# eBay/Sequence-Semantic-Embedding

Measured on AMD Instinct MI355X. Metric: encoded seqs/sec (+ query x target cosine-scores/sec, top-1 vs ref), higher is better.
Workload: dtype f32; 1 GPU; configs[1]: classification stand-in, dual-encoder LSTM H=S=256 E=50 T=32 V=32000; encode 16384 source seqs/GPU/step + cosine top-10 vs 571-target index; batch_per_gpu=16384, seq_len=32, targets=571, parallelism=dp1, weights=random-init (reference initialisers, seed 0)

## Files before the change

### sequence-semantic-embedding_amd/csrc/score_topk.hip

```cpp
#include <cstdlib>

#include "sse_kernels.h"
#include "score_exact.h"

#define SC_THREADS 512
#define SC_KC 16
#ifndef SC_PRIO_K
#define SC_PRIO_K 1
#define SC_PRIO_E 0
#endif

#ifdef SSE_SCORE_CLOCK
#include <cstdio>
__device__ long long g_score_clk[8 * 8];
#define SC_CLK_DECL long long ck_[8] = {0, 0, 0, 0, 0, 0, 0, 0}, ck_t = clock64();
#define SC_CLK(i)                   \
  {                                 \
    const long long n_ = clock64(); \
    ck_[i] += n_ - ck_t;            \
    ck_t = n_;                      \
  }
#else
#define SC_CLK_DECL
#define SC_CLK(i)
// ... 834 lines not shown
__device__ __forceinline__ float wave_max_f(float x) {
  x = fmaxf(x, dpp_f<0x128, 0xF>(x));
  x = fmaxf(x, dpp_f<0x124, 0xF>(x));
  x = fmaxf(x, dpp_f<0x122, 0xF>(x));
  x = fmaxf(x, dpp_f<0x121, 0xF>(x));
  x = fmaxf(x, dpp_f<0x142, 0xA>(x));
  x = fmaxf(x, dpp_f<0x143, 0xC>(x));
  return __int_as_float(__builtin_amdgcn_readlane(__float_as_int(x), 63));
}
template <int JMAX>
#ifdef SSE_SCORE_CLOCK
#define SI_CLK_PARAMS , long long (&ck_)[8], long long &ck_t
#define SI_CLK_ARGS , ck_, ck_t
#else
#define SI_CLK_PARAMS
#define SI_CLK_ARGS
#endif
__device__ __forceinline__ void si_select4(const SmallIndexArgs &a, const float *sc, int NP, int NT, int qt, int q0, int lane SI_CLK_PARAMS) {
  constexpr int QW = 4;
  const int J = (NT * 32 + 63) / 64;
  float v[QW][JMAX];
#pragma unroll
  for (int j = 0; j < JMAX; ++j) {
    const int row = lane + 64 * j;
#pragma unroll
    for (int c = 0; c < QW; ++c) v[c][j] = (j < J && row < NT * 32) ? sc[(q0 + c) * NP + row] : NEG_INF;
  }
  int lok[QW], hik[QW];
  float lm[QW];
  bool done[QW];
#pragma unroll
  for (int c = 0; c < QW; ++c) {
    float m = NEG_INF;
#pragma unroll
    for (int j = 0; j < JMAX; ++j) m = fmaxf(m, v[c][j]);
    lm[c] = m;
    lok[c] = si_key(-wave_max_f(-m));
    hik[c] = si_key(wave_max_f(m)) + 1;
    done[c] = false;
  }
  SC_CLK(5)
  for (;;) {
    bool all_done = true;
#pragma unroll
    for (int c = 0; c < QW; ++c) {
      const unsigned width = (unsigned)hik[c] - (unsigned)lok[c];
      const int mid = lok[c] + (int)(width >> 1);
      const int cnt = __popcll(__ballot(lm[c] >= si_val(mid)));
      const bool open = !done[c] && width > 1u;
      const bool ge = cnt >= SC_KC;
      lok[c] = (open && ge) ? mid : lok[c];
      hik[c] = (open && !ge) ? mid : hik[c];
      done[c] = !open || (ge && cnt <= 24);
      all_done = all_done && done[c];
    }
    if (all_done) break;
  }
  SC_CLK(6)
#pragma unroll
  for (int c = 0; c < QW; ++c) {
    const int query = qt * 32 + q0 + c;
    if (query < a.Q) {
      const float T = si_val(lok[c]);
      float cs = NEG_INF;
      int cr = -1, base = 0;
#pragma unroll
      for (int j = 0; j < JMAX; ++j) {
        const bool take = (j < J) & (v[c][j] >= T) & (v[c][j] > NEG_INF);
        const unsigned long long mask = __ballot(take);
        const int n = __popcll(mask);
        const int slot = base + (int)__builtin_amdgcn_mbcnt_hi((unsigned)(mask >> 32), __builtin_amdgcn_mbcnt_lo((unsigned)mask, 0u));
        const int dst = (take && slot < 63) ? slot : 63;
        const int gs = __builtin_amdgcn_ds_permute(dst * 4, __float_as_int(v[c][j]));
        const int gr = __builtin_amdgcn_ds_permute(dst * 4, lane + 64 * j);
        const bool recv = (lane >= base) & (lane < base + n) & (lane < 63);
        cs = recv ? __int_as_float(gs) : cs;
        cr = recv ? gr : cr;
        base += n;
      }
      const int nw = base < 63 ? base : 63;
      int rank = 0;
      for (int l = 0; l < nw; ++l) {
        const float os = __int_as_float(__builtin_amdgcn_readlane(__float_as_int(cs), l));
        const int orow = __builtin_amdgcn_readlane(cr, l);
        rank += ((os > cs) | ((os == cs) & (orow < cr))) ? 1 : 0;
      }
      const bool mine = lane < nw;
      if (mine && rank < SC_KC) {
        a.part_scores[(size_t)query * SC_KC + rank] = cs;
        a.part_ids[(size_t)query * SC_KC + rank] = cr;
      }
      if (lane >= nw && lane < SC_KC) {
        a.part_scores[(size_t)query * SC_KC + lane] = NEG_INF;
        a.part_ids[(size_t)query * SC_KC + lane] = -1;
      }
      const unsigned long long m16 = __ballot(mine && rank == SC_KC - 1);
      const float last = m16 ? __int_as_float(__builtin_amdgcn_readlane(__float_as_int(cs), __ffsll((long long)m16) - 1)) : NEG_INF;
      if (lane == 0) a.part_bnd[query] = (base > 63) ? __builtin_inff() : last;
    }
  }
}

template <int KGC>
__global__ __launch_bounds__(256) void score_small_index_kernel(SmallIndexArgs a) {
  extern __shared__ __attribute__((aligned(16))) float si_sc[];
  const int tid = threadIdx.x, lane = tid & 63, w = __builtin_amdgcn_readfirstlane(tid >> 6);
  const int NT = a.NT, NP = NT * 32 + 1;
  const int qt = blockIdx.x;
  float *sc = si_sc;
  SC_CLK_DECL
  f32x4 b[KGC];
  {
    const int row = qt * 32 + (lane & 31), kb = (lane >> 5) * 4;
    const float *src = a.q_rows + (size_t)(row < a.Q ? row : 0) * a.S + kb;
    const bool vec = (a.S & 3) == 0 && (reinterpret_cast<uintptr_t>(a.q_rows) & 15) == 0 && KGC * 8 <= a.S;
#pragma unroll
    for (int kg = 0; kg < KGC; ++kg) {
      f32x4 v = {0, 0, 0, 0};
      if (vec) {
        v = *reinterpret_cast<const f32x4 *>(src + kg * 8);
      } else {
#pragma unroll
        for (int e = 0; e < 4; ++e)
          if (kg * 8 + kb + e < a.S) v[e] = src[kg * 8 + e];
      }
      if (row >= a.Q) v = f32x4{0, 0, 0, 0};
      b[kg] = v;
    }
  }
  SC_CLK(0)
  for (int t = w; t < NT; t += 4) {
    const f32x4 *ap = reinterpret_cast<const f32x4 *>(a.idxp) + (size_t)t * KGC * 64 + lane;
    f32x16 acc = {0, 0, 0, 0, 0, 0, 0, 0, 0, 0, 0, 0, 0, 0, 0, 0};
    f32x4 ar[4];
#pragma unroll
    for (int d = 0; d < 4; ++d) ar[d] = ap[(d < KGC ? d : 0) * 64];
#pragma unroll
    for (int kg = 0; kg < KGC; ++kg) {
      __builtin_amdgcn_sched_barrier(0);
#pragma unroll
      for (int e = 0; e < 4; ++e) acc = __builtin_amdgcn_mfma_f32_32x32x2f32(ar[kg & 3][e], b[kg][e], acc, 0, 0, 0);
      __builtin_amdgcn_sched_barrier(0);
      ar[kg & 3] = ap[(kg + 4 < KGC ? kg + 4 : kg) * 64];
    }
    const int rb = t * 32 + 4 * (lane >> 5);
    float *col = sc + (lane & 31) * NP;
#pragma unroll
    for (int r = 0; r < 16; ++r) {
      const int row = rb + (r & 3) + 8 * (r >> 2);
      col[row] = (row < a.N) ? acc[r] : NEG_INF;
    }
  }
  SC_CLK(1)
  __syncthreads();
  SC_CLK(2)
  if (NT * 32 <= 640) {
    si_select4<10>(a, sc, NP, NT, qt, w * 8, lane SI_CLK_ARGS);
    SC_CLK(3)
    si_select4<10>(a, sc, NP, NT, qt, w * 8 + 4, lane SI_CLK_ARGS);
    SC_CLK(4)
#ifdef SSE_SCORE_CLOCK
    if (blockIdx.x == gridDim.x / 2 && lane == 0)
      for (int i = 0; i < 8; ++i) g_score_clk[w * 8 + i] = ck_[i];
#endif
  } else {
    si_select4<16>(a, sc, NP, NT, qt, w * 8, lane SI_CLK_ARGS);
    si_select4<16>(a, sc, NP, NT, qt, w * 8 + 4, lane SI_CLK_ARGS);
  }
// ... 91 lines not shown
bool score_small_index_applies(int Q, int KG, int64_t NT) {
  return Q >= 1024 && (KG == 32 || KG == 8 || KG == 7) && NT * 32 <= 1024 && (size_t)32 * (NT * 32 + 1) * sizeof(float) <= (size_t)144 * 1024;
}
hipError_t launch_score_small_index(const SmallIndexArgs &a, hipStream_t stream) {
  if (!score_small_index_applies(a.Q, a.KG, a.NT)) return hipErrorInvalidValue;
  const size_t lds = (size_t)32 * (a.NT * 32 + 1) * sizeof(float);
  const dim3 grid((a.Q + 31) / 32), block(256);
  auto go = [&](auto kernel) -> hipError_t {
    hipError_t e = hipFuncSetAttribute(reinterpret_cast<const void *>(kernel), hipFuncAttributeMaxDynamicSharedMemorySize, (int)lds);
    if (e != hipSuccess) return e;
    hipLaunchKernelGGL(kernel, grid, block, lds, stream, a);
    return hipGetLastError();
  };
  if (a.idx_x3 && a.KG != 32) return go(score_small_index_x3_kernel<4>);
  if (a.KG == 8) return go(score_small_index_kernel<8>);
  if (a.KG == 7) return go(score_small_index_kernel<7>);
  const hipError_t e32 = a.idx_x3 ? go(score_small_index_x3_kernel<16>) : go(score_small_index_kernel<32>);
  if (e32 != hipSuccess) return e32;
#ifdef SSE_SCORE_CLOCK
  if (a.Q >= 8192) {
    static int n = 0;
    if (n++ % 8 == 3) {
      long long v[64];
      (void)hipStreamSynchronize(stream);
      (void)hipMemcpyFromSymbol(v, HIP_SYMBOL(g_score_clk), sizeof v);
      for (int w = 0; w < 4; w += 3)
        fprintf(stderr, "[small index clock Q=%d NT=%d] wave %d cycles: query fragments %lld | scores (MFMA + LDS stores) %lld | barrier %lld | selection: loads + bounds %lld | bisection %lld | winners + rank + stores %lld (both batches)\n",
                a.Q, a.NT, w, v[w * 8 + 0], v[w * 8 + 1], v[w * 8 + 2], v[w * 8 + 5], v[w * 8 + 6], v[w * 8 + 3] + v[w * 8 + 4]);
    }
  }
#endif
  return hipGetLastError();
}

hipError_t launch_score_topk(const ScoreArgs &a_in, hipStream_t stream) {
  ScoreArgs a = a_in;
#ifdef SSE_SCORE_MEASURE
  {
    static const int dbg = getenv("SSE_SCORE_DBG") ? atoi(getenv("SSE_SCORE_DBG")) : 0;
    a.dbg = dbg;
  }
#endif
  if (a.KC != SC_KC) return hipErrorInvalidValue;
  if (a.q_rows && ((a.NQ != 1 && !a.COLLECT) || a.S < 1)) return hipErrorInvalidValue;
  if (a.NSPLIT > 8 && (a.NSPLIT & 7)) return hipErrorInvalidValue;
  if (a.NSPLIT < 8 && (8 % a.NSPLIT)) return hipErrorInvalidValue;
  if (a.COLLECT) {
    if (!a.lane_max && (!a.col_thr || !a.col_slot || !a.col_cnt || !a.col_buf)) return hipErrorInvalidValue;
    if (a.BF) return a.NQ == 4 ? launch_score_variant<4, true, true>(a, stream) : hipErrorInvalidValue;
    if (a.NQ == 1) return launch_score_variant<1, false, true>(a, stream);
    if (a.NQ == 2) return launch_score_variant<2, false, true>(a, stream);
    if (a.NQ == 4) return launch_score_variant<4, false, true>(a, stream);
    return hipErrorInvalidValue;
  }
  if (!a.part_bnd) return hipErrorInvalidValue;
  if (a.BF) {
    if (a.NQ == 1) return launch_score_variant<1, true, false>(a, stream);
    if (a.NQ == 2) return launch_score_variant<2, true, false>(a, stream);
    if (a.NQ == 4) return launch_score_variant<4, true, false>(a, stream);
    return hipErrorInvalidValue;
  }
  if (a.NQ == 1) return launch_score_variant<1, false, false>(a, stream);
  if (a.NQ == 2) return launch_score_variant<2, false, false>(a, stream);
  if (a.NQ == 4) return launch_score_variant<4, false, false>(a, stream);
  return hipErrorInvalidValue;
}


template <int NB>
__device__ __forceinline__ int packed_value_of_lane(int lane) {
  int v = 0;
#pragma unroll
  for (int cnt = NB, bit = 5; cnt > 1; cnt >>= 1, --bit) v = v * 2 + ((lane >> bit) & 1);
  return v;
}
template <int NB>
__device__ __forceinline__ int packed_lane_of_value(int v) {
  int lane = 0;
#pragma unroll
  for (int cnt = NB, bit = 5; cnt > 1; cnt >>= 1, --bit) lane |= ((v / (cnt / 2)) & 1) << bit;
  return lane;
}
template <int NB>
__device__ __forceinline__ double wave_exact_dot_packed(const float *qrow, const float *idxp, const double *idx64, const int64_t (&n)[NB],
                                                        int S, int KG, int lane, const float *idx_rm = nullptr) {
  static_assert(NB == 2 || NB == 4 || NB == 8, "power of two");
  double acc[NB];
#pragma unroll
  for (int b = 0; b < NB; ++b) acc[b] = 0.0;
  if (idx64) {
    for (int d = lane; d < S; d += 64) {
      double rv[NB];
#pragma unroll
      for (int b = 0; b < NB; ++b) rv[b] = idx64[(size_t)n[b] * S + d];
#pragma unroll
      for (int b = 0; b < NB; ++b) acc[b] += (double)qrow[d] * rv[b];
    }
  } else {
    for (int j = lane; j < KG * 2; j += 64) {
      const int kg = j >> 1, half = j & 1;
      f32x4 v[NB];
#pragma unroll
      for (int b = 0; b < NB; ++b)
        v[b] = idx_rm ? *reinterpret_cast<const f32x4 *>(idx_rm + (size_t)n[b] * S + j * 4)
                      : *reinterpret_cast<const f32x4 *>(idxp + (size_t)(n[b] >> 5) * KG * 256 + kg * 256 + (half * 32 + (int)(n[b] & 31)) * 4);
      const int d0 = kg * 8 + half * 4;
#pragma unroll
      for (int e = 0; e < 4; ++e)
        if (d0 + e < S) {
#pragma unroll
          for (int b = 0; b < NB; ++b) acc[b] += (double)qrow[d0 + e] * (double)v[b][e];
        }
    }
  }
  int m = 32;
#pragma unroll
  for (int cnt = NB; cnt > 1; cnt >>= 1, m >>= 1) {
    const bool up = (lane & m) != 0;
#pragma unroll
    for (int i = 0; i < cnt / 2; ++i) {
      const double send = up ? acc[i] : acc[i + cnt / 2];
      const double keep = up ? acc[i + cnt / 2] : acc[i];
      acc[i] = keep + __shfl_xor(send, m);
    }
  }
#pragma unroll
  for (; m > 0; m >>= 1) acc[0] += __shfl_xor(acc[0], m);
  return acc[0];
}

#define RS_THREADS 256
#define RS_MAXWIN 256
#define RS_MAXNC 4096
__global__ __launch_bounds__(RS_THREADS) void rescore_kernel(RescoreArgs a) {
  __shared__ int s_cnt;
  __shared__ int s_wid[RS_MAXWIN];
  __shared__ double s_ex[RS_MAXWIN];
  __shared__ float s_m[RS_THREADS / 64];
  __shared__ double s_qn[RS_THREADS / 64];
  extern __shared__ __attribute__((aligned(16))) unsigned long long s_key[];
  const int q = blockIdx.x, tid = threadIdx.x, lane = tid & 63, w = tid >> 6;
  if (a.uncert_clear && q == 0 && tid == 0) *a.uncert_clear = 0;
  if (a.q_count && q >= *a.q_count) return;
  const int qo = a.qmap ? a.qmap[q] : q;
  const float *ps = a.part_scores + (size_t)q * a.NC;
  const int32_t *pi = a.part_ids + (size_t)q * a.NC;
  const float *qrow = a.q + (size_t)q * a.S;
  const int KG = (a.S + 7) / 8;

  constexpr int PER = RS_MAXNC / RS_THREADS;
  float rs[PER];
  int ri[PER];
#pragma unroll
  for (int j = 0; j < PER; ++j) {
    const int c = tid + j * RS_THREADS;
    ri[j] = (c < a.NC) ? pi[c] : -1;
    rs[j] = (c < a.NC) ? ps[c] : NEG_INF;
  }
  float mmax = NEG_INF;
  for (int c = tid; c < a.NC / SC_KC; c += RS_THREADS) mmax = fmaxf(mmax, a.part_bnd[(size_t)q * (a.NC / SC_KC) + c]);

  {
    double v = 0.0;
    for (int d = tid; d < a.S; d += RS_THREADS) v += (double)qrow[d] * qrow[d];
#pragma unroll
    for (int o = 32; o > 0; o >>= 1) v += __shfl_xor(v, o);
    if (lane == 0) s_qn[w] = v;
  }
#pragma unroll
  for (int o = 32; o > 0; o >>= 1) mmax = fmaxf(mmax, __shfl_xor(mmax, o));
  if (lane == 0) s_m[w] = mmax;
  if (tid == 0) s_cnt = 0;

#pragma unroll
  for (int j = 0; j < PER; ++j) {
    const int c = tid + j * RS_THREADS;
    if (c < a.NC) {
      unsigned u = __float_as_uint(rs[j]);
      u = (u & 0x80000000u) ? ~u : (u | 0x80000000u);
      s_key[c] = (ri[j] < 0) ? 0ull : (((unsigned long long)u << 32) | (unsigned long long)(0xFFFFFFFFu - (unsigned)ri[j]));
    }
  }
  __syncthreads();
  const float qnorm = (float)sqrt(s_qn[0] + s_qn[1] + s_qn[2] + s_qn[3]);
  const float eps_q = a.eps * qnorm;
  mmax = fmaxf(fmaxf(s_m[0], s_m[1]), fmaxf(s_m[2], s_m[3]));
  float kth = NEG_INF;
  if (a.NC <= 256) {
    const unsigned long long key = (tid < a.NC) ? s_key[tid] : 0ull;
    int rank = 0;
    for (int j = 0; j < a.NC; ++j) rank += (s_key[j] > key) ? 1 : 0;
    float mine = (key != 0ull && rank == a.k - 1) ? rs[0] : NEG_INF;
#pragma unroll
    for (int o = 32; o > 0; o >>= 1) mine = fmaxf(mine, __shfl_xor(mine, o));
    __shared__ float s_thr[RS_THREADS / 64];
    if (lane == 0) s_thr[w] = mine;
    __syncthreads();
    kth = fmaxf(fmaxf(s_thr[0], s_thr[1]), fmaxf(s_thr[2], s_thr[3]));
  } else {
    __shared__ unsigned long long s_best[(RS_THREADS / 64) * SC_KC];
    const int nslots = a.NC / SC_KC;
    int head[RS_MAXNC / SC_KC / RS_THREADS];
#pragma unroll
    for (int j = 0; j < RS_MAXNC / SC_KC / RS_THREADS; ++j) head[j] = 0;
    for (int it = 0; it < a.k; ++it) {
      unsigned long long best = 0ull;
#pragma unroll
      for (int j = 0; j < RS_MAXNC / SC_KC / RS_THREADS; ++j) {
        const int slot = tid + j * RS_THREADS;
        if (slot < nslots && head[j] < SC_KC) {
          const unsigned long long key = s_key[slot * SC_KC + head[j]];
// ... 28 lines not shown
    for (int o = 32; o > 0; o >>= 1) {
      const unsigned long long other = __shfl_xor(kkey, o);
      kkey = other > kkey ? other : kkey;
    }
    if (kkey != 0ull) {
      unsigned u = (unsigned)(kkey >> 32);
      u = (u & 0x80000000u) ? (u & 0x7FFFFFFFu) : ~u;
      kth = __uint_as_float(u);
    }
  }

#pragma unroll
  for (int j = 0; j < PER; ++j) {
    if (ri[j] >= 0 && rs[j] >= kth - 2.0f * eps_q) {
      const int p = atomicAdd(&s_cnt, 1);
      if (p < RS_MAXWIN) s_wid[p] = ri[j];
    }
  }
  __syncthreads();
  const int nwin_all = s_cnt;
  const int nwin = min(nwin_all, RS_MAXWIN);

  for (int i0 = w * 4; i0 < nwin; i0 += (RS_THREADS / 64) * 4) {
    int64_t n[4];
#pragma unroll
    for (int c = 0; c < 4; ++c) n[c] = s_wid[min(i0 + c, nwin - 1)];
    const double tot = wave_exact_dot_packed<4>(qrow, a.idx32, a.idx64, n, a.S, KG, lane, a.idx_rm);
    const int c = packed_value_of_lane<4>(lane);
    if ((lane & 15) == 0 && i0 + c < nwin) s_ex[i0 + c] = tot;
  }
  __syncthreads();

  double theta = -__builtin_inf();
  for (int i = tid; i < nwin; i += RS_THREADS) {
    const double s = s_ex[i];
    const int64_t id = s_wid[i];
    int rank = 0;
    for (int j = 0; j < nwin; ++j) rank += before(s_ex[j], (int64_t)s_wid[j], s, id);
    if (rank < a.k) {
      a.out_scores[(size_t)qo * a.k + rank] = s;
      a.out_ids[(size_t)qo * a.k + rank] = a.id_base + id;
      if (a.host_flag) {
        a.host_scores[(size_t)qo * a.k + rank] = s;
        a.host_ids[(size_t)qo * a.k + rank] = a.id_base + id;
      }
    }
    if (rank == a.k - 1) theta = s;
  }
  if (a.host_flag) __threadfence_system();
  {
    double t = theta;
#pragma unroll
    for (int o = 32; o > 0; o >>= 1) t = fmax(t, __shfl_xor(t, o));
    __syncthreads();
    if (lane == 0) s_ex[w] = t;
    __syncthreads();
    if (tid == 0) {
      t = fmax(fmax(s_ex[0], s_ex[1]), fmax(s_ex[2], s_ex[3]));
      const bool ok = (nwin_all <= RS_MAXWIN) && (nwin >= a.k) && ((double)mmax + (double)eps_q < t);
      a.cert[qo] = ok ? 1 : 0;
      if (!ok && a.uncert) atomicAdd(a.uncert, 1);
      if (a.col_thr) a.col_thr[qo] = ok ? __builtin_inff() : __double2float_rd(t - (double)(a.eps32 * qnorm));
      if (a.col_slot) {
        a.col_slot[qo] = ok ? -1 : qo;
        a.col_cnt[qo] = 0;
      }
      if (a.host_flag) {
        a.host_cert[qo] = ok ? 1 : 0;
        if (qo == 0 && a.host_err) *a.host_err = a.err_in ? *a.err_in : 0;
        __hip_atomic_store(a.host_flag + qo, a.seq, __ATOMIC_RELEASE, __HIP_MEMORY_SCOPE_SYSTEM);
      }
    }
  }
}

#ifndef RS_NB
#define RS_NB 4
#endif
__device__ __forceinline__ double readlane_f64(double v, int l) {
  const long long b = __double_as_longlong(v);
  const int lo = __builtin_amdgcn_readlane((int)b, l), hi = __builtin_amdgcn_readlane((int)(b >> 32), l);
  return __longlong_as_double(((long long)hi << 32) | (unsigned int)lo);
}
__global__ __launch_bounds__(256) void rescore_small_kernel(RescoreArgs a) {
  const int lane = threadIdx.x & 63;
  const int q = blockIdx.x * 4 + (threadIdx.x >> 6);
  if (a.uncert_clear && blockIdx.x == 0 && threadIdx.x == 0) *a.uncert_clear = 0;
  if (q >= a.Q) return;
  if (a.q_count && q >= *a.q_count) return;
  const int qo = a.qmap ? a.qmap[q] : q;
  const float *qrow = a.q + (size_t)q * a.S;
  const int KG = (a.S + 7) / 8;
#ifdef SSE_SCORE_CLOCK
  long long rk_[6] = {0, 0, 0, 0, 0, 0}, rk_t = clock64();
#define RS_CLK(i) { const long long n_ = clock64(); rk_[i] += n_ - rk_t; rk_t = n_; }
#else
#define RS_CLK(i)
#endif
  const bool have = lane < a.NC;
  const int id = have ? a.part_ids[(size_t)q * a.NC + lane] : -1;
  const float sc = have ? a.part_scores[(size_t)q * a.NC + lane] : NEG_INF;
  const float bnd = (lane < a.NC / SC_KC) ? a.part_bnd[(size_t)q * (a.NC / SC_KC) + lane] : NEG_INF;
  double qn = 0.0;
  for (int d = lane; d < a.S; d += 64) qn += (double)qrow[d] * qrow[d];
#pragma unroll
  for (int o = 32; o > 0; o >>= 1) qn += __shfl_xor(qn, o);
  const float qnorm = (float)sqrt(qn);
  const float eps_q = a.eps * qnorm;
  RS_CLK(0)

  unsigned u = __float_as_uint(sc);
  u = (u & 0x80000000u) ? ~u : (u | 0x80000000u);
  const unsigned long long key = (id < 0) ? 0ull : (((unsigned long long)u << 32) | (unsigned long long)(0xFFFFFFFFu - (unsigned)id));
  const int key_lo = (int)(unsigned)key, key_hi = (int)(unsigned)(key >> 32);
  int rank = 0;
  for (int j = 0; j < a.NC; ++j) {
    const unsigned long long kj = ((unsigned long long)(unsigned)__builtin_amdgcn_readlane(key_hi, j) << 32) |
                                  (unsigned long long)(unsigned)__builtin_amdgcn_readlane(key_lo, j);
    rank += (kj > key) ? 1 : 0;
  }
  const unsigned long long kmask = __ballot(key != 0ull && rank == a.k - 1);
  const float kth = kmask ? __int_as_float(__builtin_amdgcn_readlane(__float_as_int(sc), __ffsll((long long)kmask) - 1)) : NEG_INF;
  const bool in_win = (id >= 0) && (sc >= kth - 2.0f * eps_q);
  float mmax = NEG_INF;
  for (int j = 0; j < a.NC / SC_KC; ++j) mmax = fmaxf(mmax, __int_as_float(__builtin_amdgcn_readlane(__float_as_int(bnd), j)));
  const unsigned long long wmask = __ballot(in_win);
  const int nwin = __popcll(wmask);
  const int mi = __popcll(wmask & ((1ull << lane) - 1ull));
  const int idm = __builtin_amdgcn_ds_permute((in_win ? mi : 63) * 4, id);
  RS_CLK(1)
  double exm = -__builtin_inf();
  for (int m0 = 0; m0 < nwin; m0 += RS_NB) {
    int64_t n[RS_NB];
#pragma unroll
    for (int c = 0; c < RS_NB; ++c) n[c] = __builtin_amdgcn_readlane(idm, (m0 + c < nwin) ? m0 + c : 0);
    const double tot = wave_exact_dot_packed<RS_NB>(qrow, a.idx32, a.idx64, n, a.S, KG, lane, a.idx_rm);
    const int want = lane - m0;
    const double got = __shfl(tot, packed_lane_of_value<RS_NB>(want & (RS_NB - 1)));
    if (want >= 0 && want < RS_NB && lane < nwin) exm = got;
  }
  RS_CLK(2)
  int r2 = 0;
  for (int j = 0; j < nwin; ++j)
    r2 += before(readlane_f64(exm, j), (int64_t)__builtin_amdgcn_readlane(idm, j), exm, (int64_t)idm) ? 1 : 0;
  const bool member = lane < nwin;
  if (member && r2 < a.k) {
    a.out_scores[(size_t)qo * a.k + r2] = exm;
    a.out_ids[(size_t)qo * a.k + r2] = a.id_base + idm;
    if (a.host_flag) {
      a.host_scores[(size_t)qo * a.k + r2] = exm;
      a.host_ids[(size_t)qo * a.k + r2] = a.id_base + idm;
    }
  }
  const unsigned long long tmask = __ballot(member && r2 == a.k - 1);
  const double theta = tmask ? readlane_f64(exm, __ffsll((long long)tmask) - 1) : -__builtin_inf();
  if (a.host_flag) __threadfence_system();
  RS_CLK(3)
#ifdef SSE_SCORE_CLOCK
  if (q == a.Q / 2 && lane == 0) {
    rk_[4] = nwin;
    for (int i = 0; i < 6; ++i) g_score_clk[i] = rk_[i];
  }
#endif
  if (lane == 0) {
    const bool ok = (nwin >= a.k) && ((double)mmax + (double)eps_q < theta);
    a.cert[qo] = ok ? 1 : 0;
    if (!ok && a.uncert) atomicAdd(a.uncert, 1);
    if (a.col_thr) a.col_thr[qo] = ok ? __builtin_inff() : __double2float_rd(theta - (double)(a.eps32 * qnorm));
    if (a.col_slot) {
      a.col_slot[qo] = ok ? -1 : qo;
      a.col_cnt[qo] = 0;
    }
    if (a.host_flag) {
      a.host_cert[qo] = ok ? 1 : 0;
      if (qo == 0 && a.host_err) *a.host_err = a.err_in ? *a.err_in : 0;
      __hip_atomic_store(a.host_flag + qo, a.seq, __ATOMIC_RELEASE, __HIP_MEMORY_SCOPE_SYSTEM);
    }
  }
}

hipError_t launch_rescore(const RescoreArgs &a, hipStream_t stream) {
  if (a.NC > RS_MAXNC) return hipErrorInvalidValue;
  if (a.NC <= 64) {
    hipLaunchKernelGGL(rescore_small_kernel, dim3((a.Q + 3) / 4), dim3(256), 0, stream, a);
#ifdef SSE_SCORE_CLOCK
    if (a.Q >= 8192) {
      static int n = 0;
      if (n++ % 8 == 3) {
        long long v[8];
        (void)hipStreamSynchronize(stream);
        (void)hipMemcpyFromSymbol(v, HIP_SYMBOL(g_score_clk), sizeof v);
        fprintf(stderr, "[rescore_small clock Q=%d NC=%d] cycles: query norm %lld | candidates, rank, k-th, window %lld | float64 dots %lld (window of %lld) | exact rank + outputs %lld\n",
                a.Q, a.NC, v[0], v[1], v[2], v[4], v[3]);
      }
    }
#endif
    return hipGetLastError();
  }
  hipLaunchKernelGGL(rescore_kernel, dim3(a.Q), dim3(RS_THREADS), (size_t)a.NC * sizeof(unsigned long long), stream, a);
  return hipGetLastError();
}

#define EX_THREADS 256
struct ExactArgs {
  const float *q;
  const float *idxp;
  const double *idx64;
  const int32_t *cert;
  double *out_scores;
  int64_t *out_ids;
  int64_t id_base, N;
  int32_t Q, S, k;
  int32_t k_off, k_total;
  unsigned long long *served;
  const int32_t *uncert;
};

__device__ __forceinline__ void exact_topk_query(const ExactArgs a, const int q, double (*s_sc)[SC_KC],
                                                 int64_t (*s_id)[SC_KC]) {
  const int tid = threadIdx.x, lane = tid & 63, w = tid >> 6;
  if (a.served && tid == 0 && a.k_off == 0) atomicAdd(a.served, 1ull);
  const float *qrow = a.q + (size_t)q * a.S;
  const int KG = (a.S + 7) / 8;
  double ls[SC_KC];
  int64_t li[SC_KC];
#pragma unroll
  for (int i = 0; i < SC_KC; ++i) {
    ls[i] = -__builtin_inf();
    li[i] = -1;
  }
  double cut_s = __builtin_inf();
  int64_t cut_id = -1;
  if (a.k_off > 0) {
    cut_s = a.out_scores[(size_t)q * a.k_total + a.k_off - 1];
    cut_id = a.out_ids[(size_t)q * a.k_total + a.k_off - 1] - a.id_base;
  }
  for (int64_t n = w; n < a.N; n += EX_THREADS / 64) {
    double s = wave_exact_dot(qrow, a.idxp, a.idx64, n, a.S, KG, lane);
    const bool after_cut = (s < cut_s) || (s == cut_s && n > cut_id);
    if (after_cut && s > ls[SC_KC - 1]) {
      int64_t id = n;
      bool ins = false;
#pragma unroll
      for (int i = 0; i < SC_KC; ++i) {
        const bool gt = ins || (s > ls[i]);
        ins = gt;
        const double tv = ls[i];
        const int64_t ti = li[i];
        ls[i] = gt ? s : tv;
        li[i] = gt ? id : ti;
        s = gt ? tv : s;
        id = gt ? ti : id;
      }
    }
  }
  if (lane == 0) {
#pragma unroll
    for (int i = 0; i < SC_KC; ++i) {
      s_sc[w][i] = ls[i];
      s_id[w][i] = li[i];
    }
  }
  __syncthreads();
  if (tid == 0) {
    unsigned pos4 = 0;
    auto pos = [&](int p) { return (int)((pos4 >> (8 * p)) & 0xFFu); };
    for (int o = 0; o < a.k; ++o) {
      int best = -1;
      for (int p = 0; p < EX_THREADS / 64; ++p) {
        if (pos(p) >= SC_KC || s_id[p][pos(p)] < 0) continue;
        if (best < 0 || before(s_sc[p][pos(p)], s_id[p][pos(p)], s_sc[best][pos(best)], s_id[best][pos(best)])) best = p;
      }
      a.out_scores[(size_t)q * a.k_total + a.k_off + o] = s_sc[best][pos(best)];
      a.out_ids[(size_t)q * a.k_total + a.k_off + o] = a.id_base + s_id[best][pos(best)];
      pos4 += 1u << (8 * best);
    }
  }
}
__global__ __launch_bounds__(EX_THREADS) void exact_topk_kernel(ExactArgs a) {
  __shared__ double s_sc[EX_THREADS / 64][SC_KC];
  __shared__ int64_t s_id[EX_THREADS / 64][SC_KC];
// ... 269 lines not shown
```

### sequence-semantic-embedding_amd/csrc/sse_api.hip

```cpp
#include <cmath>
#include <cstdarg>
#include <cstdio>
#include <cstdlib>
#include <algorithm>
#include <chrono>
#include <cstring>
#include <dlfcn.h>
#include <link.h>
#include <mutex>
#include <string>
#include <vector>

#include "../../include/sse_hip.h"
#include "sse_kernels.h"
#include "train.h"

namespace {

thread_local std::string g_create_error;

struct Variable {
  std::string name;
  int rows = 0, cols = 0;
  int64_t count = 0;
// ... 1494 lines not shown
    m2.col_thr = (const float *)h->s_cthr.p;
    m2.col_slot = (const int32_t *)h->s_cslot.p;
    m2.col_cnt = (int32_t *)h->s_ccnt.p;
    m2.col_buf = (int32_t *)h->s_cbuf.p;
    m2.col_cap = MID_CAP;
    HIPCHECK(h, launch_score_topk(m2, st));
    SelectArgs sel{q, h->idxp, h->idx64, m2.col_slot, m2.col_cnt, m2.col_buf, MID_CAP, out_s, out_i, (int32_t *)h->s_cert.p, h->idx_base,
                   Q, S, k, nullptr};
    HIPCHECK(h, launch_select_topk(sel, st));
    HIPCHECK(h, launch_exact_topk(q, h->idxp, h->idx64, (const int32_t *)h->s_cert.p, out_s, out_i, h->idx_base, h->idx_N, Q, S, k, st,
                                  counters + 2));
    if (split) *split = 0;
    return 0;
  }
  const int POOL = std::min(Q, 1024);
  if (reserve(h, h->s_qp, (size_t)QB * NQ * KG * 256 * sizeof(float))) return 1;
  if (reserve(h, h->s_ps, (size_t)Q * (bf ? NCmax : NC) * sizeof(float))) return 1;
  if (reserve(h, h->s_pi, (size_t)Q * (bf ? NCmax : NC) * sizeof(int32_t))) return 1;
  if (reserve(h, h->s_pb, (size_t)Q * (bf ? NCmax / 16 : nsplit) * sizeof(float))) return 1;
  if (reserve(h, h->s_cert, (size_t)Q * sizeof(int32_t))) return 1;
  if (reserve_collect(h, Q, POOL)) return 1;
  if (split) *split = 1;
  const bool first = phase != SCORE_REST, rest = phase != SCORE_FIRST;
  const bool rows_direct = NQ == 1;
  if (first && !rows_direct && !small_idx) {
    if (bf) HIPCHECK(h, launch_pack_rows_bf16(q, Q, S, h->s_qp.p, st));
    else HIPCHECK(h, launch_pack_rows(q, Q, S, (float *)h->s_qp.p, st));
  }
  ScoreArgs a;
  if (rows_direct) {
    a.q_rows = q;
    a.S = S;
  }
  a.BF = bf ? 1 : 0;
  a.idxp = bf ? (const float *)h->idxp16 : h->idxp;
  a.qp = (const float *)h->s_qp.p;
  a.part_scores = (float *)h->s_ps.p;
  a.part_ids = (int32_t *)h->s_pi.p;
  a.part_bnd = (float *)h->s_pb.p;
  a.N = h->idx_N;
  a.Q = Q;
  a.KG = bf ? KG16 : KG;
  a.NT = (int)NT;
  a.QT = QT;
  a.NSPLIT = nsplit;
  a.KC = 16;
  a.NQ = NQ;
  if (first) {
    if (small_idx) {
      SmallIndexArgs si{q, h->idxp, a.part_scores, a.part_ids, a.part_bnd, h->idx_N, Q, S, KG, (int)NT};
      if (small_x3) si.idx_x3 = h->idx_x3.p;
      HIPCHECK(h, launch_score_small_index(si, st));
    } else {
      HIPCHECK(h, launch_score_topk(a, st));
    }
  }
  RescoreArgs r;
  r.q = q;
  r.idx32 = h->idxp;
  r.idx64 = h->idx64;
  r.idx_rm = h->idx_rm_valid ? (const float *)h->idx_rm.p : nullptr;
  r.part_scores = a.part_scores;
  r.part_ids = a.part_ids;
  r.part_bnd = a.part_bnd;
  r.out_scores = out_s;
  r.out_ids = out_i;
  r.cert = (int32_t *)h->s_cert.p;
  r.id_base = h->idx_base;
  r.N = h->idx_N;
  r.Q = Q;
  r.S = S;
  r.NC = NC;
  r.k = k;
  const float eps32 = score_eps32(h);
  r.eps = eps32;
  r.eps32 = eps32;
  r.col_thr = (float *)h->s_cthr.p;
  if (first) h->uncert_word ^= 1;
  int32_t *const uncert = (int32_t *)(counters + 4) + h->uncert_word;
  const int follow_grid = 2 * (h->cu_count > 0 ? h->cu_count : 256);
  r.uncert = uncert;
  r.uncert_clear = (int32_t *)(counters + 4) + (h->uncert_word ^ 1);
  const bool own_slots = Q <= POOL;
  if (own_slots) {
    r.col_slot = (int32_t *)h->s_cslot.p;
    r.col_cnt = (int32_t *)h->s_ccnt.p;
  }
  if (bf) r.eps += (float)(1.02 * (1.0 / 256.0 + 1.0 / 262144.0) * h->idx_norm_max);
  if (small_x3)
    r.eps = (float)(((1.0 + 1.0 / 64.0) / 32768.0 + 2.0 * (3 * S + 2) * 5.97e-8 * (1.0 + 1.0 / 32.0)) * h->idx_norm_max);
  if (first) {
    RescoreArgs rf = r;
    if (mirror) {
      rf.host_scores = mirror->scores;
      rf.host_ids = mirror->ids;
      rf.host_cert = mirror->cert;
      rf.host_err = mirror->err;
      rf.host_flag = mirror->flag;
      rf.err_in = h->err_flag;
      rf.seq = mirror->seq;
    }
    HIPCHECK(h, launch_rescore(rf, st));
  }
  if (!rest) return 0;
  const float *qp32 = (const float *)h->s_qp.p;
  if (bf && Q > 32) {
    if (reserve(h, h->s_qp32, (size_t)QB * NQ * KG * 256 * sizeof(float))) return 1;
    if (reserve(h, h->s_qmap, (size_t)(Q + 1) * sizeof(int32_t))) return 1;
    if (reserve(h, h->s_qc, (size_t)QT * 32 * S * sizeof(float))) return 1;
    HIPCHECK(h, launch_count_uncert(r.cert, Q, counters, st));
    int32_t *qmap = (int32_t *)h->s_qmap.p, *qcount = qmap + Q;
    HIPCHECK(h, launch_compact_uncert(q, r.cert, Q, S, qmap, qcount, (float *)h->s_qc.p, st));
    if (!rows_direct) HIPCHECK(h, launch_pack_rows((const float *)h->s_qc.p, Q, S, (float *)h->s_qp32.p, st));
    ScoreArgs a2 = a;
    a2.BF = 0;
    a2.idxp = h->idxp;
    a2.qp = (const float *)h->s_qp32.p;
    if (rows_direct) a2.q_rows = (const float *)h->s_qc.p;
    a2.KG = KG;
    a2.q_count = qcount;
    a2.NSPLIT = nsplit2;
    HIPCHECK(h, launch_score_topk(a2, st));
    RescoreArgs r2 = r;
    r2.q = (const float *)h->s_qc.p;
    r2.NC = nsplit2 * 16;
    r2.eps = eps32;
    r2.qmap = qmap;
    r2.q_count = qcount;
    r2.uncert = r2.uncert_clear = nullptr;
    HIPCHECK(h, launch_rescore(r2, st));
    qp32 = (const float *)h->s_qp32.p;
  }
  if (!own_slots) {
    HIPCHECK(h, hipMemsetAsync(h->s_ccnt.p, 0, (size_t)(POOL + 1) * sizeof(int32_t), st));
    HIPCHECK(h, launch_assign_slots(r.cert, Q, POOL, (int32_t *)h->s_cslot.p, (int32_t *)h->s_ccnt.p + POOL, st));
  }
  ScoreArgs c = a;
  c.BF = 0;
  c.idxp = h->idxp;
  c.qp = qp32;
  c.q_rows = q;
  c.S = S;
  c.KG = KG;
  c.COLLECT = 1;
  c.col_thr = (const float *)h->s_cthr.p;
  c.col_slot = (const int32_t *)h->s_cslot.p;
  c.col_cnt = (int32_t *)h->s_ccnt.p;
  c.col_buf = (int32_t *)h->s_cbuf.p;
  c.col_cap = SSE_COLLECT_CAP;
  c.uncert = uncert;
  HIPCHECK(h, launch_score_topk(c, st));
  SelectArgs sel{q, h->idxp, h->idx64, c.col_slot, c.col_cnt, c.col_buf, SSE_COLLECT_CAP, out_s, out_i, r.cert, h->idx_base, Q, S, k,
                 counters + 1, uncert, follow_grid};
  HIPCHECK(h, launch_select_topk(sel, st));
  HIPCHECK(h, launch_exact_topk(q, h->idxp, h->idx64, r.cert, out_s, out_i, h->idx_base, h->idx_N, Q, S, k, st, counters + 2, uncert,
                                follow_grid));
  return 0;
}

}

extern "C" {

const char *sse_last_error(sse_handle *h) { return h ? h->err.c_str() : g_create_error.c_str(); }

int sse_create(const sse_config *cfg, sse_handle **out) {
  if (!cfg || !out) return fail(nullptr, "sse_create: null argument");
  *out = nullptr;
  int ndev = 0;
  if (hipGetDeviceCount(&ndev) != hipSuccess || ndev == 0) return fail(nullptr, "no HIP device available");
  if (cfg->device < 0 || cfg->device >= ndev) return fail(nullptr, "device %d out of range (have %d)", cfg->device, ndev);
  if (cfg->vocab_size < 2 || cfg->embedding_size < 1 || cfg->encoding_size < 1)
    return fail(nullptr, "bad model sizes V=%d E=%d S=%d", cfg->vocab_size, cfg->embedding_size, cfg->encoding_size);
  sse_handle *h = new sse_handle();
  h->cfg = *cfg;
  h->lr = cfg->learning_rate;
#define CREATE_FAIL(...)        \
  do {                          \
    fail(nullptr, __VA_ARGS__); \
    sse_destroy(h);             \
    return 1;                   \
  } while (0)
  if (hipSetDevice(cfg->device) != hipSuccess) CREATE_FAIL("hipSetDevice(%d) failed", cfg->device);
  add_var(h, "word_embedding", cfg->vocab_size, cfg->embedding_size);
  switch (cfg->network_mode) {
    case SSE_MODE_DUAL_ENCODER:
      setup_encoder(h, h->enc[0], "source_encoder", "source_encoder/src_M", cfg->src_cell_size, cfg->src_cell_size);
      setup_encoder(h, h->enc[1], "target_encoder", "target_encoder/tgt_M", cfg->tgt_cell_size, cfg->tgt_cell_size);
      break;
    case SSE_MODE_SHARED_ENCODER:
      setup_encoder(h, h->enc[0], "shared_encoder", "shared_encoder/src_M", cfg->src_cell_size, cfg->src_cell_size);
      h->enc[1] = h->enc[0];
      h->enc[1].proj = add_var(h, "shared_encoder/tgt_M", cfg->src_cell_size, cfg->encoding_size);
      h->enc[1].shares_lstm_with = 0;
      break;
    case SSE_MODE_SOURCE_ENCODER_ONLY:
      setup_encoder(h, h->enc[0], "source_only_encoder", "source_only_encoder/src_M", cfg->src_cell_size, cfg->src_cell_size);
      h->tgt_table = add_var(h, "target_embedding/tgt_seq_embedding", cfg->target_space_size, cfg->encoding_size);
      break;
    case SSE_MODE_SOURCE_ONLY_CNN: {
      static const int fs[4] = {2, 3, 4, 5}, nf[4] = {256, 128, 128, 64};
      for (int i = 0; i < 4; ++i) {
        char nm[96];
        snprintf(nm, sizeof nm, "source_only_cnn/conv-maxpool-%d/W", fs[i]);
        h->cnn_W[i] = add_var(h, nm, fs[i] * cfg->embedding_size, nf[i]);
        snprintf(nm, sizeof nm, "source_only_cnn/conv-maxpool-%d/b", fs[i]);
        h->cnn_b[i] = add_var(h, nm, 1, nf[i]);
      }
      h->cnn_M = add_var(h, "source_only_cnn/src_M", 576, cfg->encoding_size);
      h->tgt_table = add_var(h, "target_embedding/tgt_seq_embedding", cfg->target_space_size, cfg->encoding_size);
      break;
    }
    default:
      CREATE_FAIL("Unsupported network mode %d (sse_model.py:175-177)", cfg->network_mode);
  }
  for (int s = 0; s < 2; ++s)
// ... 1924 lines not shown
```

### sequence-semantic-embedding_amd/csrc/sse_kernels.h

```cpp
#pragma once
#include <hip/hip_runtime.h>
#include <stdint.h>

typedef float f32x4 __attribute__((ext_vector_type(4)));
typedef float f32x16 __attribute__((ext_vector_type(16)));

__host__ __device__ static inline int frag32_off(int r_in_tile, int k_in_group) {
  return ((((k_in_group >> 2) << 5) + r_in_tile) << 2) + (k_in_group & 3);
}

__device__ static inline int mfma_row(int reg, int lane) { return (reg & 3) + 8 * (reg >> 2) + 4 * (lane >> 5); }

static inline int round_up(int x, int m) { return (x + m - 1) / m * m; }

typedef unsigned int sse_u32x4 __attribute__((ext_vector_type(4)));
__host__ __device__ static inline unsigned short sse_bf16_rne(float f) {
  unsigned u;
  __builtin_memcpy(&u, &f, 4);
  u += 0x7FFFu + ((u >> 16) & 1u);
  return (unsigned short)(u >> 16);
}
__host__ __device__ static inline float sse_bf16_f32(unsigned short h) {
  const unsigned u = (unsigned)h << 16;
  float f;
// ... 175 lines not shown
  int32_t B, T, V, E, Ep, KGx, KGh, H, Hp, S, NTS, normalize;
  const float *pad_h = nullptr, *pad_c = nullptr;
  int32_t pad_stride = 0;
  unsigned long long *hx = nullptr;
  unsigned long long *sx = nullptr;
  uint32_t epoch = 0;
  int32_t NCL = 0;
  int32_t write_through = 0;
  int32_t plain_launch = 0;
  int32_t drop_wg = 0;
};
int lstm_cluster_ok(int E, int H, int S);
int lstm_cluster_max_rows();
size_t lstm_cluster_weight_floats(int E, int H);
size_t lstm_cluster_hx_words(int H);
size_t lstm_cluster_sx_words();
hipError_t launch_pack_lstm_cluster(const float *K, const float *b, int E, int H, float *Wc, hipStream_t stream);
hipError_t launch_lstm_cluster(const LstmClusterArgs &a, hipStream_t stream);

struct ScoreArgs {
  const float *idxp;
  const float *qp;
  float *part_scores;
  int32_t *part_ids;
  float *part_bnd;
  int64_t N;
  int32_t Q, KG, NT, QT, NSPLIT, KC;
  int32_t NQ = 4;
  int32_t thr_off = 0;
  const int32_t *q_count = nullptr;
  int32_t BF = 0;
  int32_t COLLECT = 0;
  const float *col_thr = nullptr;
  const int32_t *col_slot = nullptr;
  int32_t *col_cnt = nullptr;
  int32_t *col_buf = nullptr;
  int32_t col_cap = 0;
  float *lane_max = nullptr;
  int32_t dbg = 0;
  const float *q_rows = nullptr;
  int32_t S = 0;
  const int32_t *uncert = nullptr;
};
hipError_t launch_score_topk(const ScoreArgs &a, hipStream_t stream);
hipError_t launch_lane_max_threshold(const float *q, const float *lane_max, int Q, int S, int NV, float eps, float *col_thr,
                                     int32_t *col_slot, hipStream_t st);
#define SSE_MAX_INDEX_DIM 1024
int score_pick_nq(int Q, int S, int with_bf16);
size_t score_lds_bytes(int NQ, int KG, int BF, int COLLECT);
hipError_t launch_pack_rows_bf16(const float *rows, int64_t R, int C, void *out, hipStream_t stream);
hipError_t launch_count_uncert(const int32_t *cert, int Q, unsigned long long *count, hipStream_t st);
hipError_t launch_compact_uncert(const float *q, const int32_t *cert, int Q, int S, int32_t *qmap, int32_t *count, float *qc,
                                 hipStream_t st);
hipError_t launch_frag32_to_bf16(const float *idxp, int64_t NT, int KG, void *out, hipStream_t stream);
hipError_t launch_frag32_to_split_bf16(const float *idxp, int64_t NT, int KG, void *out, hipStream_t stream);

#define SSE_COLLECT_CAP 4096
#define SSE_MAX_SELECT_K 1024

struct RescoreArgs {
  const float *q;
  const float *idx32;
  const double *idx64;
  const float *part_scores;
  const int32_t *part_ids;
  const float *part_bnd;
  double *out_scores;
  int64_t *out_ids;
  int32_t *cert;
  int64_t id_base, N;
  int32_t Q, S, NC, k;
  float eps;
  const int32_t *qmap = nullptr, *q_count = nullptr;
  float *col_thr = nullptr;
  float eps32 = 0.0f;
  int32_t *col_slot = nullptr, *col_cnt = nullptr;
  double *host_scores = nullptr;
  int64_t *host_ids = nullptr;
  int32_t *host_cert = nullptr, *host_flag = nullptr, *host_err = nullptr;
  const int32_t *err_in = nullptr;
  int32_t seq = 0;
  const float *idx_rm = nullptr;
  int32_t *uncert = nullptr, *uncert_clear = nullptr;
};
hipError_t launch_rescore(const RescoreArgs &a, hipStream_t stream);

struct SmallIndexArgs {
  const float *q_rows;
  const float *idxp;
  float *part_scores;
  int32_t *part_ids;
  float *part_bnd;
  int64_t N;
  int32_t Q, S, KG, NT;
  const void *idx_x3 = nullptr;
};
bool score_small_index_applies(int Q, int KG, int64_t NT);
hipError_t launch_score_small_index(const SmallIndexArgs &a, hipStream_t stream);

struct RankArgs {
  const float *q;
  const int32_t *pair_q;
  const int64_t *pair_id;
  const double *pair_score_in;
  const float *idxp;
  const double *idx64;
  int64_t *out_before;
  double *out_score;
  double *thr64;
  float *lo, *hi;
  unsigned long long *sure;
  int32_t *band_cnt, *band_buf;
  int32_t band_cap;
  const int32_t *bad;
  unsigned long long *counters;
  int64_t id_base, N;
  int32_t S, KG, NT, P, NSPLIT, NQ;
  float eps32;
};
hipError_t launch_rank_validate(const int32_t *pair_q, const int64_t *pair_id, int64_t L, int Q, int need_row, int64_t id_base,
                                int64_t N, int32_t *bad, int32_t *err_flag, hipStream_t st);
hipError_t launch_score_rank(const RankArgs &a, hipStream_t st);

struct AboveArgs {
  const float *q;
  const int32_t *pair_q;
  const double *pair_thr;
  const float *idxp;
  const double *idx64;
  float *lo, *hi;
  unsigned long long *sure;
  int32_t *band_cnt, *band_buf;
  int32_t band_cap;
  const int32_t *bad;
  int32_t *err_flag;
  unsigned long long *counters;
  int64_t *counts;
  const int64_t *offsets;
  const int64_t *total;
  int32_t *ovf;
  unsigned long long *cursor;
  int64_t *out_ids;
  int64_t cap;
  int64_t id_base, N;
  int32_t S, KG, NT, P, NSPLIT, NQ, emit;
  float eps32;
};
#define SSE_ABOVE_SORT_CAP 8192
hipError_t launch_above_validate(const int32_t *pair_q, int64_t L, int Q, int32_t *bad, int32_t *err_flag, hipStream_t st);
hipError_t launch_score_above(const AboveArgs &a, hipStream_t st);
hipError_t launch_above_scan(int64_t *offsets, int64_t L, const int32_t *bad, hipStream_t st);
struct AboveListArgs {
  const float *q;
  const int32_t *pair_q;
  const float *idxp;
  const double *idx64;
  const int64_t *offsets;
  const unsigned long long *cursor;
  int64_t *ids;
  double *scores;
  int64_t *scratch_ids;
  double *scratch_scores;
  const int32_t *bad;
  int32_t *err_flag;
  unsigned long long *counters;
  int64_t L, cap, id_base, N;
// ... 120 lines not shown
```

Baseline: 7.607 million seqs/s.

## Specialize small-index rescore for pre-sorted top-16 and assign collect slots inline

Adds a SORTED variant of the small-index rescore kernel. Because the small-index scorer already emits candidates in rank order, the kernel reads the k-th score and the bound directly and drops the O(NC) readlane rank loop and the compaction permute. The exact double dots now load 8 candidate rows at once and overlap the second batch's loads with the first batch's reduction. Collect slots are assigned from the uncertain-count atomic inside rescore, which removes a memset and the separate assign_slots launch. The in-wave tie-break also uses lane order instead of reading row ids. Risks are wrong slot or tie ordering if the sorted assumption fails, and extra register pressure from the 8-row batch.

```diff
diff --git a/sequence-semantic-embedding_amd/csrc/score_topk.hip b/sequence-semantic-embedding_amd/csrc/score_topk.hip
--- a/sequence-semantic-embedding_amd/csrc/score_topk.hip
+++ b/sequence-semantic-embedding_amd/csrc/score_topk.hip
@@ -940,8 +940,7 @@
       int rank = 0;
       for (int l = 0; l < nw; ++l) {
         const float os = __int_as_float(__builtin_amdgcn_readlane(__float_as_int(cs), l));
-        const int orow = __builtin_amdgcn_readlane(cr, l);
-        rank += ((os > cs) | ((os == cs) & (orow < cr))) ? 1 : 0;
+        rank += ((os > cs) | ((os == cs) & (l < lane))) ? 1 : 0;
       }
       const bool mine = lane < nw;
       if (mine && rank < SC_KC) {
@@ -1199,6 +1198,24 @@
   return lane;
 }
 template <int NB>
+__device__ __forceinline__ double wave_packed_reduce(double (&acc)[NB], int lane) {
+  int m = 32;
+#pragma unroll
+  for (int cnt = NB; cnt > 1; cnt >>= 1, m >>= 1) {
+    const bool up = (lane & m) != 0;
+#pragma unroll
+    for (int i = 0; i < cnt / 2; ++i) {
+      const double lo = acc[i], hi = acc[i + cnt / 2];
+      const double send = up ? lo : hi;
+      const double keep = up ? hi : lo;
+      acc[i] = keep + __shfl_xor(send, m);
+    }
+  }
+#pragma unroll
+  for (; m > 0; m >>= 1) acc[0] += __shfl_xor(acc[0], m);
+  return acc[0];
+}
+template <int NB>
 __device__ __forceinline__ double wave_exact_dot_packed(const float *qrow, const float *idxp, const double *idx64, const int64_t (&n)[NB],
                                                         int S, int KG, int lane, const float *idx_rm = nullptr) {
   static_assert(NB == 2 || NB == 4 || NB == 8, "power of two");
@@ -1230,20 +1247,7 @@
         }
     }
   }
-  int m = 32;
-#pragma unroll
-  for (int cnt = NB; cnt > 1; cnt >>= 1, m >>= 1) {
-    const bool up = (lane & m) != 0;
-#pragma unroll
-    for (int i = 0; i < cnt / 2; ++i) {
-      const double send = up ? acc[i] : acc[i + cnt / 2];
-      const double keep = up ? acc[i + cnt / 2] : acc[i];
-      acc[i] = keep + __shfl_xor(send, m);
-    }
-  }
-#pragma unroll
-  for (; m > 0; m >>= 1) acc[0] += __shfl_xor(acc[0], m);
-  return acc[0];
+  return wave_packed_reduce<NB>(acc, lane);
 }
 
 #define RS_THREADS 256
@@ -1438,6 +1442,7 @@
   const int lo = __builtin_amdgcn_readlane((int)b, l), hi = __builtin_amdgcn_readlane((int)(b >> 32), l);
   return __longlong_as_double(((long long)hi << 32) | (unsigned int)lo);
 }
+template <bool SORTED>
 __global__ __launch_bounds__(256) void rescore_small_kernel(RescoreArgs a) {
   const int lane = threadIdx.x & 63;
   const int q = blockIdx.x * 4 + (threadIdx.x >> 6);
@@ -1465,35 +1470,93 @@
   const float eps_q = a.eps * qnorm;
   RS_CLK(0)
 
-  unsigned u = __float_as_uint(sc);
-  u = (u & 0x80000000u) ? ~u : (u | 0x80000000u);
-  const unsigned long long key = (id < 0) ? 0ull : (((unsigned long long)u << 32) | (unsigned long long)(0xFFFFFFFFu - (unsigned)id));
-  const int key_lo = (int)(unsigned)key, key_hi = (int)(unsigned)(key >> 32);
-  int rank = 0;
-  for (int j = 0; j < a.NC; ++j) {
-    const unsigned long long kj = ((unsigned long long)(unsigned)__builtin_amdgcn_readlane(key_hi, j) << 32) |
-                                  (unsigned long long)(unsigned)__builtin_amdgcn_readlane(key_lo, j);
-    rank += (kj > key) ? 1 : 0;
-  }
-  const unsigned long long kmask = __ballot(key != 0ull && rank == a.k - 1);
-  const float kth = kmask ? __int_as_float(__builtin_amdgcn_readlane(__float_as_int(sc), __ffsll((long long)kmask) - 1)) : NEG_INF;
-  const bool in_win = (id >= 0) && (sc >= kth - 2.0f * eps_q);
-  float mmax = NEG_INF;
-  for (int j = 0; j < a.NC / SC_KC; ++j) mmax = fmaxf(mmax, __int_as_float(__builtin_amdgcn_readlane(__float_as_int(bnd), j)));
-  const unsigned long long wmask = __ballot(in_win);
-  const int nwin = __popcll(wmask);
-  const int mi = __popcll(wmask & ((1ull << lane) - 1ull));
-  const int idm = __builtin_amdgcn_ds_permute((in_win ? mi : 63) * 4, id);
+  float kth, mmax;
+  bool in_win;
+  unsigned long long wmask;
+  int nwin, idm;
+  if constexpr (SORTED) {
+    const int idk = __builtin_amdgcn_readlane(id, a.k - 1);
+    kth = idk >= 0 ? __int_as_float(__builtin_amdgcn_readlane(__float_as_int(sc), a.k - 1)) : NEG_INF;
+    in_win = (id >= 0) && (sc >= kth - 2.0f * eps_q);
+    mmax = __int_as_float(__builtin_amdgcn_readlane(__float_as_int(bnd), 0));
+    wmask = __ballot(in_win);
+    nwin = __popcll(wmask);
+    idm = id;
+  } else {
+    unsigned u = __float_as_uint(sc);
+    u = (u & 0x80000000u) ? ~u : (u | 0x80000000u);
+    const unsigned long long key = (id < 0) ? 0ull : (((unsigned long long)u << 32) | (unsigned long long)(0xFFFFFFFFu - (unsigned)id));
+    const int key_lo = (int)(unsigned)key, key_hi = (int)(unsigned)(key >> 32);
+    int rank = 0;
+    for (int j = 0; j < a.NC; ++j) {
+      const unsigned long long kj = ((unsigned long long)(unsigned)__builtin_amdgcn_readlane(key_hi, j) << 32) |
+                                    (unsigned long long)(unsigned)__builtin_amdgcn_readlane(key_lo, j);
+      rank += (kj > key) ? 1 : 0;
+    }
+    const unsigned long long kmask = __ballot(key != 0ull && rank == a.k - 1);
+    kth = kmask ? __int_as_float(__builtin_amdgcn_readlane(__float_as_int(sc), __ffsll((long long)kmask) - 1)) : NEG_INF;
+    in_win = (id >= 0) && (sc >= kth - 2.0f * eps_q);
+    mmax = NEG_INF;
+    for (int j = 0; j < a.NC / SC_KC; ++j) mmax = fmaxf(mmax, __int_as_float(__builtin_amdgcn_readlane(__float_as_int(bnd), j)));
+    wmask = __ballot(in_win);
+    nwin = __popcll(wmask);
+    const int mi = __popcll(wmask & ((1ull << lane) - 1ull));
+    idm = __builtin_amdgcn_ds_permute((in_win ? mi : 63) * 4, id);
+  }
   RS_CLK(1)
   double exm = -__builtin_inf();
-  for (int m0 = 0; m0 < nwin; m0 += RS_NB) {
-    int64_t n[RS_NB];
-#pragma unroll
-    for (int c = 0; c < RS_NB; ++c) n[c] = __builtin_amdgcn_readlane(idm, (m0 + c < nwin) ? m0 + c : 0);
-    const double tot = wave_exact_dot_packed<RS_NB>(qrow, a.idx32, a.idx64, n, a.S, KG, lane, a.idx_rm);
-    const int want = lane - m0;
-    const double got = __shfl(tot, packed_lane_of_value<RS_NB>(want & (RS_NB - 1)));
-    if (want >= 0 && want < RS_NB && lane < nwin) exm = got;
+  if (SORTED && !a.idx64) {
+    constexpr int NB2 = 2 * RS_NB;
+    const bool act = lane < KG * 2;
+    const int d0 = (lane >> 1) * 8 + (lane & 1) * 4;
+    f32x4 v[NB2];
+    double acc[2][RS_NB];
+    auto load_rows = [&](int m0) __attribute__((always_inline)) {
+#pragma unroll
+      for (int c = 0; c < NB2; ++c) {
+        const int64_t n = __builtin_amdgcn_readlane(idm, (m0 + c < nwin) ? m0 + c : 0);
+        const float *p = a.idx_rm ? a.idx_rm + (size_t)n * a.S + lane * 4
+                                  : a.idx32 + (size_t)(n >> 5) * KG * 256 + (lane >> 1) * 256 + ((lane & 1) * 32 + (int)(n & 31)) * 4;
+        v[c] = act ? *reinterpret_cast<const f32x4 *>(p) : f32x4{0, 0, 0, 0};
+      }
+    };
+    auto dots = [&]() __attribute__((always_inline)) {
+#pragma unroll
+      for (int c = 0; c < NB2; ++c) acc[c / RS_NB][c % RS_NB] = 0.0;
+#pragma unroll
+      for (int e = 0; e < 4; ++e)
+        if (d0 + e < a.S) {
+#pragma unroll
+          for (int c = 0; c < NB2; ++c) acc[c / RS_NB][c % RS_NB] += (double)qrow[d0 + e] * (double)v[c][e];
+        }
+    };
+    auto reduce_place = [&](int m0) __attribute__((always_inline)) {
+      const double t0 = wave_packed_reduce<RS_NB>(acc[0], lane), t1 = wave_packed_reduce<RS_NB>(acc[1], lane);
+      const int want = lane - m0;
+      const int src = packed_lane_of_value<RS_NB>(want & (RS_NB - 1));
+      const double g0 = __shfl(t0, src), g1 = __shfl(t1, src);
+      if (want >= 0 && want < NB2 && lane < nwin) exm = want < RS_NB ? g0 : g1;
+    };
+    if (nwin > 0) {
+      load_rows(0);
+      dots();
+      if (nwin > NB2) load_rows(NB2);
+      reduce_place(0);
+      if (nwin > NB2) {
+        dots();
+        reduce_place(NB2);
+      }
+    }
+  } else {
+    for (int m0 = 0; m0 < nwin; m0 += RS_NB) {
+      int64_t n[RS_NB];
+#pragma unroll
+      for (int c = 0; c < RS_NB; ++c) n[c] = __builtin_amdgcn_readlane(idm, (m0 + c < nwin) ? m0 + c : 0);
+      const double tot = wave_exact_dot_packed<RS_NB>(qrow, a.idx32, a.idx64, n, a.S, KG, lane, a.idx_rm);
+      const int want = lane - m0;
+      const double got = __shfl(tot, packed_lane_of_value<RS_NB>(want & (RS_NB - 1)));
+      if (want >= 0 && want < RS_NB && lane < nwin) exm = got;
+    }
   }
   RS_CLK(2)
   int r2 = 0;
@@ -1521,11 +1584,18 @@
   if (lane == 0) {
     const bool ok = (nwin >= a.k) && ((double)mmax + (double)eps_q < theta);
     a.cert[qo] = ok ? 1 : 0;
-    if (!ok && a.uncert) atomicAdd(a.uncert, 1);
+    int nth = -1;
+    if (!ok && a.uncert) nth = atomicAdd(a.uncert, 1);
     if (a.col_thr) a.col_thr[qo] = ok ? __builtin_inff() : __double2float_rd(theta - (double)(a.eps32 * qnorm));
     if (a.col_slot) {
-      a.col_slot[qo] = ok ? -1 : qo;
-      a.col_cnt[qo] = 0;
+      if (a.slot_pool > 0) {
+        const int slot = (nth >= 0 && nth < a.slot_pool) ? nth : -1;
+        a.col_slot[qo] = slot;
+        if (slot >= 0) a.col_cnt[slot] = 0;
+      } else {
+        a.col_slot[qo] = ok ? -1 : qo;
+        a.col_cnt[qo] = 0;
+      }
     }
     if (a.host_flag) {
       a.host_cert[qo] = ok ? 1 : 0;
@@ -1538,7 +1608,13 @@
 hipError_t launch_rescore(const RescoreArgs &a, hipStream_t stream) {
   if (a.NC > RS_MAXNC) return hipErrorInvalidValue;
   if (a.NC <= 64) {
-    hipLaunchKernelGGL(rescore_small_kernel, dim3((a.Q + 3) / 4), dim3(256), 0, stream, a);
+    if (a.slot_pool > 0 && !(a.uncert && a.col_slot && a.col_cnt)) return hipErrorInvalidValue;
+    if (a.sorted16) {
+      if (a.NC != SC_KC || a.k < 1 || a.k > SC_KC || a.S > 256 || a.qmap || a.q_count) return hipErrorInvalidValue;
+      hipLaunchKernelGGL(rescore_small_kernel<true>, dim3((a.Q + 3) / 4), dim3(256), 0, stream, a);
+    } else {
+      hipLaunchKernelGGL(rescore_small_kernel<false>, dim3((a.Q + 3) / 4), dim3(256), 0, stream, a);
+    }
 #ifdef SSE_SCORE_CLOCK
     if (a.Q >= 8192) {
       static int n = 0;
@@ -1553,6 +1629,7 @@
 #endif
     return hipGetLastError();
   }
+  if (a.sorted16 || a.slot_pool > 0) return hipErrorInvalidValue;
   hipLaunchKernelGGL(rescore_kernel, dim3(a.Q), dim3(RS_THREADS), (size_t)a.NC * sizeof(unsigned long long), stream, a);
   return hipGetLastError();
 }
diff --git a/sequence-semantic-embedding_amd/csrc/sse_api.hip b/sequence-semantic-embedding_amd/csrc/sse_api.hip
--- a/sequence-semantic-embedding_amd/csrc/sse_api.hip
+++ b/sequence-semantic-embedding_amd/csrc/sse_api.hip
@@ -1600,10 +1600,13 @@
   r.uncert = uncert;
   r.uncert_clear = (int32_t *)(counters + 4) + (h->uncert_word ^ 1);
   const bool own_slots = Q <= POOL;
-  if (own_slots) {
+  const bool rescore_slots = small_idx && !own_slots;
+  if (own_slots || rescore_slots) {
     r.col_slot = (int32_t *)h->s_cslot.p;
     r.col_cnt = (int32_t *)h->s_ccnt.p;
   }
+  if (rescore_slots) r.slot_pool = POOL;
+  if (small_idx) r.sorted16 = 1;
   if (bf) r.eps += (float)(1.02 * (1.0 / 256.0 + 1.0 / 262144.0) * h->idx_norm_max);
   if (small_x3)
     r.eps = (float)(((1.0 + 1.0 / 64.0) / 32768.0 + 2.0 * (3 * S + 2) * 5.97e-8 * (1.0 + 1.0 / 32.0)) * h->idx_norm_max);
@@ -1649,7 +1652,7 @@
     HIPCHECK(h, launch_rescore(r2, st));
     qp32 = (const float *)h->s_qp32.p;
   }
-  if (!own_slots) {
+  if (!own_slots && !rescore_slots) {
     HIPCHECK(h, hipMemsetAsync(h->s_ccnt.p, 0, (size_t)(POOL + 1) * sizeof(int32_t), st));
     HIPCHECK(h, launch_assign_slots(r.cert, Q, POOL, (int32_t *)h->s_cslot.p, (int32_t *)h->s_ccnt.p + POOL, st));
   }
diff --git a/sequence-semantic-embedding_amd/csrc/sse_kernels.h b/sequence-semantic-embedding_amd/csrc/sse_kernels.h
--- a/sequence-semantic-embedding_amd/csrc/sse_kernels.h
+++ b/sequence-semantic-embedding_amd/csrc/sse_kernels.h
@@ -281,6 +281,7 @@
   int32_t seq = 0;
   const float *idx_rm = nullptr;
   int32_t *uncert = nullptr, *uncert_clear = nullptr;
+  int32_t sorted16 = 0, slot_pool = 0;
 };
 hipError_t launch_rescore(const RescoreArgs &a, hipStream_t stream);
 
```

Result: no change. 7.660 million seqs/s, median of 6 (+0.7%).
